# ethz-asl/multipoint

Measured on AMD Instinct MI355X. Metric: image-pairs/sec (detect+desc+match) @ 480x640, higher is better.
Workload: dtype f32

## Files before the change

multipoint_amd/csrc/api.hip:

```cpp
#include "host.h"

using namespace mp_host;

namespace {

bool debug_switch(const char* key, int* value = nullptr, int dflt = 1)
{
    const char* e = getenv("MP_DEBUG");
    if (!e) return false;
    const size_t kl = std::strlen(key);
    for (const char* q = e; *q;) {
        while (*q == ',' || *q == ' ') ++q;
        const char* end = q;
        while (*end && *end != ',') ++end;
        if ((size_t)(end - q) >= kl && std::strncmp(q, key, kl) == 0 && (q[kl] == '=' || q + kl == end || q[kl] == ' ')) {
            if (value) *value = q[kl] == '=' ? atoi(q + kl + 1) : dflt;
            return true;
        }
        q = end;
    }
    return false;
}

int kfd_num_xcc(const char* bus_id)
// ... 69 lines not shown
        char bus[64] = {0};
        if (hipDeviceGetPCIBusId(bus, sizeof bus, device) == hipSuccess) nxcd = kfd_num_xcc(bus);
        if (nxcd <= 0) nxcd = ncu >= 32 ? ncu / 32 : 1;
        int v = 0;
        if (debug_switch("ncu", &v) && v > 0 && v <= ncu) ncu = v;
        if (debug_switch("nxcd", &v) && v > 0) nxcd = v;
    }
    if (ncu < 1 || nxcd < 1 || (nxcd & (nxcd - 1)) != 0 || nxcd > ncu)
        return fail(h, MP_EINVAL, "mp_create: unsupported machine shape: " + std::to_string(ncu) + " compute units in " +
                                      std::to_string(nxcd) + " XCDs (the XCD count must be a power of two <= the CU count)");
    int xcd_shift = 0;
    while ((1 << xcd_shift) < nxcd) ++xcd_shift;
    DebugSwitches d;
    int v = 0;
    d.winograd = !debug_switch("no_winograd");
    if (debug_switch("wino43", &v) && v == 0) d.wino43 = false;
    if (debug_switch("wino43_gen", &v) && v >= 0 && v <= 2) d.wino43_gen = v;
    d.fuse_first = !debug_switch("no_fuse");
    d.fuse43 = !debug_switch("no_fuse43");
    d.head_fuse = !debug_switch("no_head_fuse");
    d.vin = !debug_switch("no_vin");
    d.planar = !debug_switch("no_planar");
    d.xplanar = d.planar && !debug_switch("no_xplanar");
    if (debug_switch("persist_min_items", &v) && v > 0) d.persist = v;
    if (debug_switch("no_persist")) d.persist = 0;
    if (debug_switch("splitk_max", &v) && v >= 1 && v <= 8) d.splitk_max = v;
    d.f16_res = !debug_switch("f16_no_res");
    d.f16_fuse1 = !debug_switch("f16_no_fuse1");
    if (debug_switch("f16_res_groups", &v) && v == 2) d.f16_res_groups = 2;
    mp_handle* hh = new mp_handle(device, ncu, xcd_shift, d);
    if (hipHostMalloc(reinterpret_cast<void**>(&hh->pinned), 4096) != hipSuccess) {
        delete hh;
        return fail(h, MP_ENOMEM, "mp_create: hipHostMalloc failed");
    }
    *out = hh;
    return MP_OK;
}

void mp_destroy(mp_handle* h)
{
    if (!h) return;
    (void)hipSetDevice(h->device);
    int* pinned = h->pinned;
    const std::vector<ProfEntry> events = std::move(h->prof_entries);
    delete h;
    if (pinned) (void)hipHostFree(pinned);
// ... 31 lines not shown
```

multipoint_amd/csrc/conv_wino43.hip:

```cpp
#include "mp_common.h"
#include "mp_device.h"
#include "mp_tile.h"

#include <algorithm>
#include <type_traits>

MP_TIMING_TABLE(g_timing_q, 256 * 8, mp_debug_read_timing_wino43)
MP_TIMING_HEIGHT(g_timing_q_sel, 480, mp_debug_select_height_wino43)

namespace {

constexpr int NPIX = 18 * 34;
constexpr int UC4 = 4;
constexpr int VB4 = UC4 * 32 * 36;
constexpr int UB4 = UC4 * 64 * 36;
constexpr int NRB = (NPIX + 63) / 64;
constexpr int RB4 = NRB * 64 * 4;
constexpr int SW4 = 8 * 36 * 2;


template <int LEAD = 0>
__device__ __forceinline__ void dma16(const float* sbase, unsigned voff_bytes, unsigned lds_byte)
{
    lds_dma<4, LEAD, 0>(sbase, voff_bytes, lds_byte);
}

template <bool POOL, bool BNF, int TC4, bool F1, bool SPLIT = false, bool VIN = false>
__global__ __launch_bounds__(512, 2) void conv_wino43_kernel(const ConvParams p)
{
    static_assert(!(F1 && SPLIT), "the fused first block is never split");
    static_assert(!(VIN && (F1 || SPLIT)), "pre-transformed input: plain launches only");
    constexpr int TR4 = 32 / TC4;
    constexpr int OY = 4 * TR4, OX = 4 * TC4;
    constexpr int PY = OY + 2, PX = OX + 2;
    static_assert(PY * PX == NPIX, "item shape");
    __shared__ __attribute__((aligned(16))) float Vs[(VIN ? 4 : 2) * VB4];
    __shared__ __attribute__((aligned(16))) float Us[2 * UB4];
    __shared__ __attribute__((aligned(16))) float raw[VIN ? 256 : 3 * RB4 + 256];
    __shared__ __attribute__((aligned(16))) float scr[VIN ? 4 : 8 * SW4];
    __shared__ __attribute__((aligned(16))) float prm[(POOL && !SPLIT ? 6 : 3) * 64];

    const int tid = threadIdx.x;
    const int lane = tid & 63;
    const int wave = __builtin_amdgcn_readfirstlane(tid >> 6);
    const int tb = wave & 1, cb = wave >> 1;
    const int NC = SPLIT ? (p.cin / UC4) >> p.ks_shift : p.cin / UC4;

    const XcdRange xr = xcd_range(p.nitems, p.xcd_shift);
    const int stride = xr.stride, item_end = xr.item_end;
    int item = xr.item;
    if (item >= item_end) return;

    struct Where { int slice, img, y0, x0, tile; const float* in_base; };
    auto decode = [&](int it) __attribute__((always_inline)) -> Where {
        Where w{};
        const int tile = (int)udiv((unsigned)it, p.magic_slices, (unsigned)p.nslices);
        w.slice = it - tile * p.nslices;
        w.tile = tile;
        const int trow = (int)udiv((unsigned)tile, p.magic_tx, (unsigned)p.tiles_x);
        const int tx = tile - trow * p.tiles_x;
        const int bi = (int)udiv((unsigned)trow, p.magic_ty, (unsigned)p.tiles_y);
        const int ty = trow - bi * p.tiles_y;
        w.img = p.img_list ? p.img_list[bi] : bi;
        w.y0 = ty * OY; w.x0 = tx * OX;
        w.in_base = p.in_planar ? p.in + (long long)w.img * (p.cin / 4) * p.H * p.W * 4
                                : p.in + (long long)w.img * p.H * p.W * p.in_cstride + p.in_coff;
        if constexpr (SPLIT)
            w.in_base += (long long)((w.slice & ((1 << p.ks_shift) - 1)) * NC) * (p.in_planar ? (long long)p.H * p.W * 4 : UC4);
        return w;
    };

    const int pix_stride = p.in_planar ? 4 : p.in_cstride;
    const long long unit_stride = p.in_planar ? (long long)p.H * p.W * 4 : UC4;
    const int x_shift = p.in_planar == MP_LAYOUT_XPLANAR ? 2 : 0, x_mask = p.in_planar == MP_LAYOUT_XPLANAR ? 3 : 0;
    const int row_stride = p.W * pix_stride;
    auto pixel_off = [&](int y, int x) __attribute__((always_inline)) -> int {
        return y * row_stride + (x >> x_shift) * pix_stride + (x & x_mask) * p.W;
    };
    unsigned rvoff[2];
    bool roff_rel = false;
    auto raw_offsets = [&](const Where& w) __attribute__((always_inline)) -> const float* {
// ... 447 lines not shown
                unit(c + 2, std::false_type{}, VB1{}, VS3{});
                unit(c + 3, std::false_type{}, VB0{}, VB0{});
            }
            unit(NC - 3, std::false_type{}, VB1{}, VB1{});
            unit(NC - 2, std::false_type{}, VB0{}, VS2{});
            unit(NC - 1, std::false_type{}, VB1{}, VS3{});
        } else {
        unit(0, std::true_type{}, VB0{}, VB0{});
        for (int c = 1; c + 1 < NC; c += 2) {
            unit(c, std::false_type{}, VB1{}, VB1{});
            unit(c + 1, std::false_type{}, VB0{}, VB0{});
        }
        unit(NC - 1, std::false_type{}, VB1{}, VB1{});
        }

        MP_CLOCK(t_e0);
        MP_CLOCK_ADD(3, t_item, t_e0);
        if constexpr (F1) { if (item_next + stride < item_end) patch_dma(decode(item_next + stride), cur_par); }
        const int tl = tb * 16 + (lane & 15);
        const int cl = cb * 16 + 4 * (lane >> 4);
        const f32x4 b4 = *reinterpret_cast<const f32x4*>(&prm[cl]);
        const f32x4 s4 = *reinterpret_cast<const f32x4*>(&prm[64 + cl]);
        const f32x4 t4 = *reinterpret_cast<const f32x4*>(&prm[128 + cl]);
        const int oy = cur.y0 + 4 * (tl / TC4), ox = cur.x0 + 4 * (tl % TC4);
        const int ch0 = (SPLIT ? cur.slice >> p.ks_shift : cur.slice) * 64 + cl;
        const int cs = p.out_cstride;
        constexpr int NO = POOL ? 2 : 4;
        f32x2 keep[NO][NO];
        if constexpr (SPLIT) {
            unsigned long long* const part = reinterpret_cast<unsigned long long*>(p.split_scratch) + (long long)item * (2 * 16 * 512) + tid;
#pragma unroll
            for (int h = 0; h < 2; ++h) {
                f32x2 tcol[4][6];
#pragma unroll
                for (int j = 0; j < 6; ++j) {
                    f32x2 m[6], y[4];
#pragma unroll
                    for (int i = 0; i < 6; ++i) m[i] = f32x2{acc[6 * i + j][2 * h], acc[6 * i + j][2 * h + 1]};
                    at6s(m, y);
#pragma unroll
                    for (int a = 0; a < 4; ++a) tcol[a][j] = y[a];
                }
#pragma unroll
                for (int a = 0; a < 4; ++a) {
                    f32x2 y[4];
                    at6s(tcol[a], y);
#pragma unroll
// ... 62 lines not shown
            for (int a = 0; a < 4; ++a) {
                f32x2 y[4];
                at6s(tcol[a], y);
#pragma unroll
                for (int b = 0; b < 4; ++b) {
                    f32x2 v = w43_add_bias(y[b], a, b, bb);
                    if (BNF) { v = v * ss + tt; v = f32x2{relu_bits(v[0]), relu_bits(v[1])}; }
                    else { v = f32x2{relu_bits(v[0]), relu_bits(v[1])}; v = v * ss + tt; }
                    yv[a][b] = v;
                }
            }
#pragma unroll
            for (int a = 0; a < NO; ++a)
#pragma unroll
                for (int b = 0; b < NO; ++b) res[a][b] = yv[a][b];
            }
            if (h == 0) {
#pragma unroll
                for (int a = 0; a < NO; ++a)
#pragma unroll
                    for (int b = 0; b < NO; ++b) keep[a][b] = res[a][b];
            } else {
                const int Ho = POOL ? p.H >> 1 : p.H, Wo = POOL ? p.W >> 1 : p.W;
                const int py0 = POOL ? oy >> 1 : oy, px0 = POOL ? ox >> 1 : ox;
                const bool xpl = !POOL && p.out_planar == MP_LAYOUT_XPLANAR;
                char* const img_base = reinterpret_cast<char*>(
                    p.out_planar ? p.out + (long long)cur.img * (p.cout / 4) * Ho * Wo * 4
                                 : p.out + (long long)cur.img * Ho * Wo * cs + p.out_coff);
                const unsigned ps = xpl ? (unsigned)Wo * 4u : p.out_planar ? 16u : (unsigned)cs * 4u;
                const unsigned rs = p.out_planar ? (unsigned)Wo * 16u : (unsigned)Wo * ps;
                const unsigned o0 = xpl ? (unsigned)(((ch0 >> 2) * Ho + py0) * Wo * 4 + px0) * 4u
                                  : p.out_planar ? (unsigned)(((ch0 >> 2) * Ho + py0) * Wo + px0) * 16u
                                                 : (unsigned)((py0 * Wo + px0) * cs + ch0) * 4u;
                if (oy < p.H && ox < p.W && ch0 < p.cout) {
#pragma unroll
                    for (int a = 0; a < NO; ++a)
#pragma unroll
                        for (int b = 0; b < NO; ++b) {
                            const f32x4 v = {keep[a][b][0], keep[a][b][1], res[a][b][0], res[a][b][1]};
                            *reinterpret_cast<f32x4*>(img_base + (o0 + (unsigned)a * rs + (unsigned)b * ps)) = v;
                        }
                }
            }
        }
        }
        MP_CLOCK(t_e1);
        MP_CLOCK_ADD(2, t_e0, t_e1);
#ifdef MP_TIMING
        tsum[7] += 1;
        if (!has_next && tid == 0 && t_on)
            for (int i = 0; i < 8; ++i) g_timing_q[blockIdx.x * 8 + i] = tsum[i];
#endif
        if (!has_next) { dma_wait(); return; }
        if (next_slice != cur.slice) {
            __syncthreads();
            load_prm(next_slice);
        }
        item = item_next;
        cur = decode(item);
        cur_par ^= 1;
        up = unext;
    }
}

template <int TC4>
__global__ __launch_bounds__(256) void wino43_vprod_kernel(const ConvParams p, long long ntb)
{
    constexpr int TR4 = 32 / TC4, OY = 4 * TR4, OX = 4 * TC4;
    __shared__ __attribute__((aligned(16))) float st[19456];
    const int ncp = p.cin >> 1, NC = p.cin / UC4;
    const int TL = 256 / ncp;
    const int RS = TL * 36 + 4;
    const int groups = 32 / TL;
    const int tid = threadIdx.x;
    const int cp = tid % ncp, tlc = tid / ncp;
    const long long tb = (long long)blockIdx.x / groups;
    const int t0 = ((int)((long long)blockIdx.x % groups)) * TL, t = t0 + tlc;
    (void)ntb;
    const int tx = (int)(tb % p.tiles_x);
    const long long trow = tb / p.tiles_x;
    const int ty = (int)(trow % p.tiles_y);
    const int bi = (int)(trow / p.tiles_y);
    const int img = p.img_list ? p.img_list[bi] : bi;
    const int wy = ty * OY + 4 * (t / TC4) - 1, wx = tx * OX + 4 * (t % TC4) - 1;
    const float* const base = p.in + (long long)img * p.H * p.W * p.in_cstride + p.in_coff + 2 * cp;
    int gx[6];
#pragma unroll
    for (int j = 0; j < 6; ++j) gx[j] = reflect_clamp(wx + j, p.W);
    f32x2 r[6][6];
#pragma unroll
    for (int j = 0; j < 6; ++j) {
        f32x2 d[6], o[6];
#pragma unroll
        for (int i = 0; i < 6; ++i)
            d[i] = *reinterpret_cast<const f32x2*>(base + ((long long)reflect_clamp(wy + i, p.H) * p.W + gx[j]) * p.in_cstride);
        bt6(d, o);
#pragma unroll
        for (int i = 0; i < 6; ++i) r[i][j] = o[i];
    }
    float* const dst0 = st + (2 * cp) * RS + tlc * 36;
    float* const dst1 = dst0 + RS;
#pragma unroll
    for (int i = 0; i < 6; i += 2) {
        f32x2 a[6], b[6];
        bt6(r[i], a);
        bt6(r[i + 1], b);
        *reinterpret_cast<f32x4*>(dst0 + 6 * i) = f32x4{a[0][0], a[1][0], a[2][0], a[3][0]};
// ... 9 lines not shown
    for (int i = tid; i < total4; i += 256) {
        const int row = i / q4, w = i - row * q4;
        *reinterpret_cast<f32x4*>(gbase + (long long)row * (32 * 36) + w * 4) = *reinterpret_cast<const f32x4*>(st + row * RS + w * 4);
    }
}

template <bool POOL, int TC4, bool F1 = false, bool SPLIT = false>
int launch_q(const ConvParams& p, hipStream_t s)
{
    constexpr int OY = 4 * (32 / TC4), OX = 4 * TC4;
    ConvParams q = p;
    if (SPLIT) q.nslices = p.nslices << p.ks_shift;
    q.tiles_x = (p.W + OX - 1) / OX; q.tiles_y = (p.H + OY - 1) / OY;
    const long long nitems = (long long)p.B * q.tiles_x * q.tiles_y * q.nslices;
    if (nitems <= 0) return 0;
    if (tile_items(q, nitems)) return 1;
    const unsigned grid = persistent_grid(nitems, p.ncu, p.xcd_shift);
    const ConvParams& pp = q;
    if (p.bn_first) hipLaunchKernelGGL((conv_wino43_kernel<POOL, true, TC4, F1, SPLIT>), dim3(grid), dim3(512), 0, s, pp);
    else hipLaunchKernelGGL((conv_wino43_kernel<POOL, false, TC4, F1, SPLIT>), dim3(grid), dim3(512), 0, s, pp);
    return 0;
}

template <int TC4>
int launch_vin(const ConvParams& p, hipStream_t s)
{
    constexpr int OY = 4 * (32 / TC4), OX = 4 * TC4;
    ConvParams q = p;
    q.tiles_x = (p.W + OX - 1) / OX; q.tiles_y = (p.H + OY - 1) / OY;
    const long long ntb = (long long)p.B * q.tiles_x * q.tiles_y, nitems = ntb * q.nslices;
    if (nitems <= 0) return 0;
    if (tile_items(q, nitems)) return 1;
    const ConvParams& pp = q;
    const int tl = 256 / (p.cin / 2);
    hipLaunchKernelGGL((wino43_vprod_kernel<TC4>), dim3((unsigned)(ntb * (32 / tl))), dim3(256), 0, s, pp, ntb);
    const unsigned grid = persistent_grid(nitems, p.ncu, p.xcd_shift);
    if (p.bn_first) hipLaunchKernelGGL((conv_wino43_kernel<false, true, TC4, false, false, true>), dim3(grid), dim3(512), 0, s, pp);
    else hipLaunchKernelGGL((conv_wino43_kernel<false, false, TC4, false, false, true>), dim3(grid), dim3(512), 0, s, pp);
    return 0;
}

template <bool POOL, bool SPLIT = false>
int launch_shape(const ConvParams& p, hipStream_t s)
{
    const long long wide = (long long)((p.W + 31) / 32) * ((p.H + 15) / 16), tall = (long long)((p.W + 15) / 16) * ((p.H + 31) / 32);
    return tall < wide ? launch_q<POOL, 4, false, SPLIT>(p, s) : launch_q<POOL, 8, false, SPLIT>(p, s);
}

}

bool conv_wino43_supports(const ConvParams& p)
{
    return !p.pad_zero && p.cin % 8 == 0 && p.cout % 4 == 0 && p.H % 4 == 0 && p.W % 4 == 0 && p.H >= 4 && p.W >= 4 &&
           p.in_cstride % 4 == 0 && p.in_coff % 4 == 0 && p.out_cstride % 4 == 0 && p.out_coff % 4 == 0;
}

long long conv_wino43_vglobal_floats(const ConvParams& p)
{
    const long long wide = (long long)((p.W + 31) / 32) * ((p.H + 15) / 16), tall = (long long)((p.W + 15) / 16) * ((p.H + 31) / 32);
    return (long long)p.B * std::min(wide, tall) * (p.cin / UC4) * VB4;
}

long long conv_wino43_items(const ConvParams& p)
{
    const long long wide = (long long)((p.W + 31) / 32) * ((p.H + 15) / 16), tall = (long long)((p.W + 15) / 16) * ((p.H + 31) / 32);
    return (long long)p.B * std::min(wide, tall) * p.nslices;
}

int launch_conv_wino43(const ConvParams& p, bool pool, hipStream_t s, bool fuse_first)
{
    if (p.out_planar == MP_LAYOUT_XPLANAR && pool) return 2;
    if ((p.in_planar == MP_LAYOUT_XPLANAR || p.out_planar == MP_LAYOUT_XPLANAR) && p.ks_shift > 0) return 2;
    if (fuse_first) return pool && p.cin == 64 ? launch_q<true, 8, true>(p, s) : 2;
    if (p.vglobal) {
        if (pool || p.ks_shift > 0 || p.cin % 16 != 0 || p.in_planar || p.cin > 256 || 256 % (p.cin / 2) != 0 || (p.cin / 2) < 8) return 2;
        const long long wide = (long long)((p.W + 31) / 32) * ((p.H + 15) / 16), tall = (long long)((p.W + 15) / 16) * ((p.H + 31) / 32);
        return tall < wide ? launch_vin<4>(p, s) : launch_vin<8>(p, s);
    }
    if (p.ks_shift > 0) {
        const int ncs = (p.cin / 4) >> p.ks_shift;
        if (ncs < 4 || (ncs & 1) || (ncs << p.ks_shift) * 4 != p.cin || !p.split_scratch) return 2;
        const int rc = pool ? launch_shape<true, true>(p, s) : launch_shape<false, true>(p, s);
        return rc ? rc : launch_split_reduce(p, 1, pool, s);
    }
    return pool ? launch_shape<true>(p, s) : launch_shape<false>(p, s);
}
```

multipoint_amd/csrc/forward.hip:

```cpp
#include "host.h"

using namespace mp_host;

namespace {

int pick_mbw(int H, int W)
{
    long long best = -1;
    int arg = 32;
    for (int mbw : {32, 16, 8}) {
        const int tw = mbw, th = 256 / mbw;
        const long long area = (long long)((H + th - 1) / th) * th * ((W + tw - 1) / tw) * tw;
        if (best < 0 || area < best) { best = area; arg = mbw; }
    }
    return arg;
}

void prof_begin(mp_handle* h, const char* name, double flop, hipStream_t s)
{
    if (!h->prof) return;
    if (h->prof_used == h->prof_entries.size()) {
        ProfEntry e{};
        (void)hipEventCreate(&e.a); (void)hipEventCreate(&e.b);
        h->prof_entries.push_back(e);
// ... 9 lines not shown
    (void)hipEventRecord(h->prof_entries[h->prof_used].b, s);
    ++h->prof_used;
}

int launch_failed(mp_handle* h, int code, const char* name, int B, int H, int W)
{
    const std::string layer = std::string("mp_forward: layer ") + name;
    if (code == 1)
        return fail(h, MP_EINVAL, layer + " has too many work items for one launch (B=" + std::to_string(B) + ", " +
                                      std::to_string(H) + "x" + std::to_string(W) + "): split the batch");
    return fail(h, MP_EINVAL, layer + ": the selected convolution kernel does not cover this layer shape (" + std::to_string(H) +
                                  "x" + std::to_string(W) + ")");
}


enum class Kernel { direct, wino43, wino43b, f16, f16_res, f16_res_slices };

struct ConvLaunch {
    Kernel kernel = Kernel::direct;
    bool fuse_first = false;
    int in_planar = MP_LAYOUT_NHWC, out_planar = MP_LAYOUT_NHWC;
    int ks_shift = 0;
    bool vin = false;
};

struct EncoderPlan { ConvLaunch conv[7]; };

Kernel wino43_kind(const mp_handle* h, const ConvLayer& L, int H, int W, int in_cstride, int in_coff, int out_cstride, int out_coff)
{
    if (!(L.taps == 9 && L.u43pack && h->policy.wino43)) return Kernel::direct;
    ConvParams q{};
    q.pad_zero = h->cfg.reflection_pad ? 0 : 1; q.cin = L.cin; q.cout = L.cout; q.H = H; q.W = W;
    q.in_cstride = in_cstride; q.in_coff = in_coff; q.out_cstride = out_cstride; q.out_coff = out_coff;
    if (h->policy.wino43_gen != 2 && conv_wino43_supports(q)) return Kernel::wino43;
    if (h->policy.wino43_gen != 1 && conv_wino43b_supports(q)) return Kernel::wino43b;
    return Kernel::direct;
}

void plan_split_vin(const mp_handle* h, const ConvLayer& L, int B, int H, int W, int fwd_batch, ConvLaunch& c)
{
    if ((c.kernel != Kernel::wino43 && c.kernel != Kernel::wino43b) || c.fuse_first) return;
    if (fwd_batch <= 2 && h->policy.splitk_max > 1) {
        ConvParams q{};
        q.B = B; q.H = H; q.W = W; q.nslices = L.nslices;
        const long long items = conv_wino43_items(q);
        const int units = L.cin / 4;
        int ks = 0;
        while ((items << (ks + 1)) <= h->ncu && (2 << ks) <= h->policy.splitk_max && (units >> (ks + 1)) >= 4 &&
               ((units >> (ks + 1)) & 1) == 0 && ((units >> (ks + 1)) << (ks + 1)) == units) ++ks;
        if (ks > 0 && items <= 1024) c.ks_shift = ks;
    }
    c.vin = c.kernel == Kernel::wino43 && !L.pool && c.ks_shift == 0 && !c.in_planar && L.cin % 16 == 0 && L.cin <= 256 &&
            256 % (L.cin / 2) == 0 && L.cin >= 16 && h->dbg.vin && L.nslices >= 4;
}

Kernel f16_kind(const mp_handle* h, const ConvLayer& L, int in_cstride, int in_coff, bool fuse_first)
{
    ConvParamsH q{};
    q.cin = L.cin; q.cout = L.cout; q.nslices = L.nslices; q.in_cstride = in_cstride; q.in_coff = in_coff;
    if (h->dbg.f16_res && conv_f16_res_supports(q, L.taps)) return Kernel::f16_res;
    if (h->dbg.f16_res && !fuse_first && L.taps == 9 && L.cin == 64 && L.nslices > 1 && L.cout == 64 * L.nslices)
        return Kernel::f16_res_slices;
    return Kernel::f16;
}

EncoderPlan plan_encoder(const mp_handle* h, const Encoder& E, int nb, int fwd_batch, int H, int W)
{
    EncoderPlan P;
    if (h->cfg.mixed_precision) {
        const ConvLayer& L0 = E.conv[0];
        P.conv[0].fuse_first = h->dbg.f16_res && h->dbg.f16_fuse1 && h->cfg.reflection_pad && !E.first_pool && L0.pool &&
                               L0.cin == 64 && L0.cout == 64 && L0.nslices == 1;
        for (int i = 0; i < E.nconv; ++i) P.conv[i].kernel = f16_kind(h, E.conv[i], E.conv[i].cin, 0, P.conv[i].fuse_first);
        return P;
    }
    for (int i = 0, hh = E.first_pool ? H / 2 : H, ww = E.first_pool ? W / 2 : W; i < E.nconv; ++i) {
// ... 51 lines not shown
    p.scale = L.scale; p.shift = L.shift; p.img_list = img_list;
    if (c.fuse_first) {
        p.img = images; p.w1 = f16 ? first->w_h : first->w; p.b1 = f16 ? first->bias_h : first->bias;
        p.s1 = first->scale; p.t1 = first->shift;
    }
    if constexpr (f16) {
        p.wpack = L.wpack_h; p.bias = L.bias_h;
        p.dummy = static_cast<_Float16*>(h->f16_dummy.p);
        p.res_groups = h->dbg.f16_res_groups;
    } else {
        p.wpack = c.kernel == Kernel::direct ? L.wpack : L.u43pack; p.bias = L.bias;
        p.relu = L.relu ? 1 : 0;
        p.persist = h->dbg.persist;
        p.in_planar = c.in_planar; p.out_planar = c.out_planar;
        if (c.fuse_first && c.kernel != Kernel::direct) {
            p.wpack = L.u43pack_f1; p.bias = L.bias_f1; p.w1 = first->w_f1; p.b1 = first->bias_f1; p.s1 = nullptr; p.t1 = nullptr;
        }
        if (c.ks_shift) {
            const int rc = ensure(h, h->split_ws, (size_t)(conv_wino43_items(p) << c.ks_shift) * (2 * 16 * 512 * 8));
            if (rc) return rc;
            p.ks_shift = c.ks_shift; p.split_scratch = static_cast<float*>(h->split_ws.p);
        }
        if (c.vin) {
            if (ensure(h, h->vin_ws, (size_t)conv_wino43_vglobal_floats(p) * 4) == MP_OK) p.vglobal = static_cast<float*>(h->vin_ws.p);
            else { (void)hipGetLastError(); h->err.clear(); }
        }
    }
    prof_begin(h, c.fuse_first ? "enc.conv1+2" : L.name,
               2.0 * L.taps * L.cin * L.cout * (double)B * H * W + (c.fuse_first ? 2.0 * 9 * 64 * (double)B * H * W : 0.0), s);
    int big = 0;
    if constexpr (f16) {
        if (c.kernel == Kernel::f16_res) {
            big = launch_conv_f16_res(p, mbw, L.pool, s);
        } else if (c.kernel == Kernel::f16_res_slices) {
            for (int sl = 0; sl < L.nslices && !big; ++sl) {
                ConvParamsH q = p;
                q.wpack = p.wpack + (size_t)sl * 36 * 2 * 64 * 8;
                q.bias = p.bias + 64 * sl; q.scale = p.scale + 64 * sl; q.shift = p.shift + 64 * sl;
                q.out_coff = out_coff + 64 * sl; q.cout = 64; q.nslices = 1;
                big = conv_f16_res_supports(q, L.taps) ? launch_conv_f16_res(q, mbw, L.pool, s) : 2;
            }
        } else {
            big = launch_conv_f16(p, L.taps, mbw, L.pool, s);
        }
    } else {
        big = c.kernel == Kernel::wino43b ? launch_conv_wino43b(p, L.pool, s)
// ... 85 lines not shown
        for (int i = 0; i < E.nconv; ++i) {
            const ConvLayer& L = E.conv[i];
            if ((rc = run_conv(h, L, plan.conv[i], src, L.cin, 0, i == E.nconv - 1 ? X : dst, L.cout, 0, nb, hh, ww, list, s,
                               &E.first, images))) return rc;
            if (L.pool) { hh /= 2; ww /= 2; }
            T* t = src; src = dst; dst = t;
        }
    }

    const int Hc = H / 8, Wc = W / 8, lstride = f16 ? 128 : 80;
    const long long npx = (long long)B * Hc * Wc;
    const int D = h->cfg.descriptor_size;
    const int hc = h->head_channels;
    const int headc = h->cfg.descriptor_head ? 2 * hc : hc;
    const int encc = h->heads3.cin;
    ConvLaunch c3, c1x1;
    if constexpr (f16) {
        c3.kernel = f16_kind(h, h->heads3, encc, 0, false);
        c1x1.kernel = Kernel::f16;
    } else {
        c3.kernel = wino43_kind(h, h->heads3, Hc, Wc, encc, 0, headc, 0);
        plan_split_vin(h, h->heads3, B, Hc, Wc, B, c3);
    }
    if ((rc = run_conv(h, h->heads3, c3, X, encc, 0, P, headc, 0, B, Hc, Wc, nullptr, s))) return rc;
    if (h->dbg.head_fuse && (!f16 || prob || logits || desc)) {
        typename std::conditional<f16, HeadTailParamsH, HeadTailParams>::type t{};
        t.x = P; t.xstride = headc; t.K = hc;
        if constexpr (f16) {
            t.wdet = h->det1.wpack_h; t.bdet = h->det1.bias_h; t.wdesc = h->desc1.wpack_h; t.bdesc = h->desc1.bias_h;
        } else {
            t.wdet = h->det1.wpack; t.bdet = h->det1.bias; t.wdesc = h->desc1.wpack; t.bdesc = h->desc1.bias;
        }
        t.sdet = h->det1.scale; t.tdet = h->det1.shift; t.sdesc = h->desc1.scale; t.tdesc = h->desc1.shift;
        t.D = D; t.npx = npx; t.B = B; t.Hc = Hc; t.Wc = Wc;
        t.prob = prob; t.logits_nchw = logits; t.desc = desc;
        t.softmax_mode = h->cfg.softmax_mode; t.normalize = h->cfg.normalize_descriptors ? 1 : 0; t.ncu = h->ncu;
        prof_begin(h, "heads.tail", 2.0 * hc * (65.0 + (desc ? D : 0)) * (double)npx, s);
        int miss;
        if constexpr (f16) miss = launch_head_tail_f16(t, s); else miss = launch_head_tail(t, s);
        prof_end(h, s);
        if (!miss) return launch_status(h);
        if (h->prof) --h->prof_used;
        if (!h->head_fallback_noted) {
            h->head_fallback_noted = true;
            fprintf(stderr, "[multipoint_hip] note: fused head tail not instantiated for %d head channels / descriptor size %d: "
                            "using the separate 1x1 convolution, softmax and normalisation launches\n", hc, D);
        }
    }
    if ((rc = run_conv(h, h->det1, c1x1, P, headc, 0, Lg, lstride, 0, B, Hc, Wc, nullptr, s))) return rc;
    if (prob || logits) {
        prof_begin(h, "det.softmax_shuffle", 0.0, s);
        if constexpr (f16) launch_det_post_f16(Lg, lstride, B, Hc, Wc, prob, logits, h->cfg.softmax_mode, s);
        else launch_det_post(Lg, lstride, B, Hc, Wc, prob, logits, h->cfg.softmax_mode, s);
        prof_end(h, s);
    }
    if (desc) {
        T* raw;
        if constexpr (f16) raw = R; else raw = desc;
// ... 246 lines not shown
```

multipoint_amd/csrc/head_tail.hip:

```cpp
#include "mp_common.h"
#include "mp_device.h"

#include <type_traits>

namespace {

__device__ __forceinline__ float acc_rd(float a)
{
    float x;
    asm volatile("v_accvgpr_read_b32 %0, %1" : "=v"(x) : "a"(a));
    return x;
}
template <int ND>
__global__ __launch_bounds__(256) void head_tail_kernel(const HeadTailParams p)
{
    constexpr int NT = 3 + ND;
    constexpr int NP = 96 + 32 * ND;
    constexpr int WCH = 4 * NT * 256;
    constexpr int XCH = 2 * 4 * 256;
    __shared__ __attribute__((aligned(16))) float wl[2 * WCH];
    __shared__ __attribute__((aligned(16))) float xl[2 * 4 * XCH];
    __shared__ __attribute__((aligned(16))) float prm[3 * NP];
    const int tid = threadIdx.x, lane = tid & 63;
    const int wave = __builtin_amdgcn_readfirstlane(tid >> 6);
    const int pl = lane & 31, hf = lane >> 5;
    for (int i = tid; i < NP; i += 256) {
        const bool det = i < 96;
        const int c = det ? i : i - 96;
        prm[i] = det ? p.bdet[c] : p.bdesc[c];
        prm[NP + i] = det ? p.sdet[c] : p.sdesc[c];
        prm[2 * NP + i] = det ? p.tdet[c] : p.tdesc[c];
    }

    const long long ntiles = (p.npx + 127) / 128;
    long long tile = blockIdx.x;
    long long px = 0;
    bool valid = false;
    unsigned xoff = 0, xoff_next = 0;
    const float *xbase = p.x, *xbase_next = p.x;
    auto place = [&](long long t, unsigned& off, const float*& base) __attribute__((always_inline)) {
        const long long q = (t * 4 + wave) * 32 + pl;
        off = (unsigned)(((q < p.npx ? q : p.npx - 1) - t * 128) * p.xstride + hf * 4) * 4u;
        base = p.x + t * 128 * p.xstride;
    };
    place(tile, xoff, xbase);
    const int nchunks = p.K >> 5;
    const unsigned wl_lds = (unsigned)(size_t)wl, xl_lds = (unsigned)(size_t)xl + (unsigned)wave * (XCH * 4u);

    auto chunk_dma = [&](int c, int buf, int j, bool next_tile) __attribute__((always_inline)) {
        if (j < NT) {
            const int nb = j < 3 ? j : j - 3;
            const float* w = j < 3 ? p.wdet : p.wdesc;
            const float* src = w + (((((long long)(nb >> 1) * nchunks + c) * 4 + wave) * 2 + (nb & 1)) * 64) * 4;
            lds_dma<4, 0, 0>(src, (unsigned)lane * 16u, wl_lds + (unsigned)(buf * WCH + (wave * NT + j) * 256) * 4u);
        } else {
            const int q = j - NT, part = q >> 2, g = q & 3;
            if (ND == 0 && part == 1) return;
            lds_dma<4, 0, 0>((next_tile ? xbase_next : xbase) + part * p.K + c * 32 + g * 8, next_tile ? xoff_next : xoff,
                             xl_lds + (unsigned)(buf * 4 * XCH + (part * 4 + g) * 256) * 4u);
        }
    };

#pragma unroll
    for (int j = 0; j < NT + 8; ++j) chunk_dma(0, 0, j, false);
    dma_wait();
    __syncthreads();

    for (;;) {
    const bool has_next = tile + gridDim.x < ntiles;
    if (has_next) place(tile + gridDim.x, xoff_next, xbase_next);
    px = (tile * 4 + wave) * 32 + pl;
    valid = px < p.npx;
    f32x16 acc[NT];
#pragma unroll
    for (int t = 0; t < NT; ++t)
#pragma unroll
        for (int r = 0; r < 16; ++r) acc[t][r] = 0.f;

    auto chunk = [&](int c, auto buf_tag, bool prefetch, bool next_tile) __attribute__((always_inline)) {
        constexpr int buf = decltype(buf_tag)::value;
        const float* const wb = wl + buf * WCH + lane * 4;
        const float* const xb = xl + wave * XCH + buf * 4 * XCH + lane * 4;
// ... 100 lines not shown
            if (p.normalize) {
                ss += __shfl_xor(ss, 32);
                const float rd = 1.0f / fmaxf(sqrtf(ss), 1e-12f);
#pragma unroll
                for (int i = 0; i < ND * 4; ++i) dv[i] = dv[i] * rd;
            }
            if (valid) {
                float* o = p.desc + px * (32 * ND) + 4 * hf;
#pragma unroll
                for (int t = 0; t < ND; ++t)
#pragma unroll
                    for (int q = 0; q < 4; ++q) *reinterpret_cast<f32x4*>(o + 32 * t + 8 * q) = dv[4 * t + q];
            }
        }
    }
    if (!has_next) return;
    tile += gridDim.x;
    xoff = xoff_next; xbase = xbase_next;
    }
}

}

int launch_head_tail(const HeadTailParams& p, hipStream_t s)
{
    if (p.K % 64 != 0 || p.npx <= 0) return 1;
    const int D = p.desc ? p.D : 0;
    const long long tiles = (p.npx + 127) / 128;
    const dim3 grid((unsigned)(tiles < p.ncu ? tiles : p.ncu)), block(256);
    switch (D) {
    case 0: hipLaunchKernelGGL(head_tail_kernel<0>, grid, block, 0, s, p); return 0;
    case 64: hipLaunchKernelGGL(head_tail_kernel<2>, grid, block, 0, s, p); return 0;
    case 128: hipLaunchKernelGGL(head_tail_kernel<4>, grid, block, 0, s, p); return 0;
    case 256: hipLaunchKernelGGL(head_tail_kernel<8>, grid, block, 0, s, p); return 0;
    default: return 1;
    }
}
```

multipoint_amd/csrc/host.h:

```cpp
#pragma once
#include "../../include/multipoint_hip.h"
#include "mp_common.h"

#include <cmath>
#include <cstdio>
#include <cstdlib>
#include <cstring>
#include <map>
#include <string>
#include <type_traits>
#include <vector>

namespace mp_host {

inline std::string g_create_error;

struct DevBuf {
    void* p = nullptr;
    size_t bytes = 0;
    DevBuf(void* p_ = nullptr, size_t bytes_ = 0) : p(p_), bytes(bytes_) {}
    DevBuf(DevBuf&& o) noexcept : p(o.p), bytes(o.bytes) { o.p = nullptr; o.bytes = 0; }
    ~DevBuf() { if (p) (void)hipFree(p); }
};

// ... 17 lines not shown

struct Encoder {
    FirstLayer first;
    ConvLayer conv[7];
    int nconv = 7;
    bool first_pool = false;
};

struct BnLayer {
    std::string name;
    int channels = 0;
    float *gamma = nullptr, *beta = nullptr;
    long long offset = 0;
};

struct ProfEntry {
    const char* name;
    hipEvent_t a, b;
    double flop;
};

struct DebugSwitches {
    bool winograd = true, wino43 = true, fuse_first = true, fuse43 = true, head_fuse = true, vin = true, planar = true;
    bool xplanar = true, f16_res = true, f16_fuse1 = true;
    int wino43_gen = 0, persist = 8, splitk_max = 8, f16_res_groups = 3;
};

struct ConvPolicy {
    bool direct = false;
    bool wino43 = true;
    int wino43_gen = 0;
    int splitk_max = 8;
};

struct MiRefine {
    void* workspace = nullptr;
    MiLaunch L{};
    int P = 0, normalized = 0;
    double sigma = 0.0;
    long long smooth_stride = 0;
    unsigned* counts = nullptr;
    float* warped = nullptr;
    double *smooth_a = nullptr, *smooth_b = nullptr, *cand = nullptr, *values = nullptr;
    const double* reg_init = nullptr;
    MiNmState* state = nullptr;
    int* nact = nullptr;
};
// ... 92 lines not shown
```

multipoint_amd/csrc/mp_common.h:

```cpp
#pragma once
#include <hip/hip_runtime.h>
#include <stdint.h>

typedef float f32x16 __attribute__((ext_vector_type(16)));
typedef float f32x4 __attribute__((ext_vector_type(4)));
typedef float f32x2 __attribute__((ext_vector_type(2)));

#define MP_WAVE 64

enum { MP_LAYOUT_NHWC = 0, MP_LAYOUT_PLANAR = 1, MP_LAYOUT_XPLANAR = 2 };

struct ConvParams {
    const float* in;
    float* out;
    const float* wpack;
    const float* bias;
    const float* scale;
    const float* shift;
    const int* img_list;
    const float* img;
    const float *w1, *b1, *s1, *t1;
    int B, H, W;
    int in_cstride, in_coff, cin;
    int out_cstride, out_coff, cout;
    int nslices;
    int tiles_x, tiles_y;
    int pad_zero;
    int bn_first;
    int relu;
    long long total_px;
    unsigned magic_slices, magic_tx, magic_ty;
    int nitems;
    int persist;
    int in_planar, out_planar;
    int ncu, xcd_shift;
    int ks_shift;
    float* split_scratch;
    float* vglobal;
};

struct XcdRange { int item, item_end, stride; };
__device__ __forceinline__ XcdRange xcd_range(int nitems, int xcd_shift)
{
    const int nxcd = 1 << xcd_shift;
    const int per_xcd = (nitems + nxcd - 1) >> xcd_shift;
    const int xcd = (int)blockIdx.x & (nxcd - 1);
    XcdRange r;
    r.stride = (int)gridDim.x >> xcd_shift;
    r.item_end = min((xcd + 1) * per_xcd, nitems);
    r.item = xcd * per_xcd + ((int)blockIdx.x >> xcd_shift);
    return r;
}
inline unsigned persistent_grid(long long nitems, int ncu, int xcd_shift, int per_cu = 1)
{
    const long long nxcd = 1ll << xcd_shift;
    const long long full = ((long long)ncu * per_cu) / nxcd * nxcd;
    const long long need = (nitems + nxcd - 1) / nxcd * nxcd;
    return (unsigned)(need < full ? need : full);
}

struct Conv1Params {
// ... 58 lines not shown
    r[4] = pk_fnma_k<1>(t3, K_AB, t2);
    r[5] = pk_fma_k<0>(d[1], K_PS, pk_fnma_k<1>(d[3], K_PS, d[5]));
}
static_assert(MP_W43_B == 2 * MP_W43_A, "at6s() needs b = 2a");
__device__ __forceinline__ void at6s(const f32x2 m[6], f32x2 z[4])
{
    constexpr float a3 = (float)(MP_W43_A * MP_W43_A * MP_W43_A);
    const f32x2 s1 = m[1] + m[2], d1 = m[1] - m[2], s2 = m[3] + m[4], d2 = m[3] - m[4];
    z[0] = (m[0] + s1) + s2;
    z[1] = __builtin_elementwise_fma(d2, f32x2{2.f, 2.f}, d1);
    z[2] = __builtin_elementwise_fma(s2, f32x2{4.f, 4.f}, s1);
    z[3] = __builtin_elementwise_fma(__builtin_elementwise_fma(d2, f32x2{8.f, 8.f}, d1), f32x2{a3, a3}, m[5]);
}
constexpr float w43_sigma(int r) { return r == 1 ? (float)MP_W43_A : r == 2 ? (float)(MP_W43_A * MP_W43_A) : 1.f; }
constexpr float w43_out_scale(int r, int c) { return w43_sigma(r) * w43_sigma(c); }
__device__ __forceinline__ f32x2 w43_add_bias(f32x2 z, int r, int c, f32x2 bias)
{
    const float k = w43_out_scale(r, c);
    return k == 1.f ? z + bias : __builtin_elementwise_fma(z, f32x2{k, k}, bias);
}
bool conv_wino43_supports(const ConvParams& p);
long long conv_wino43_items(const ConvParams& p);
long long conv_wino43_vglobal_floats(const ConvParams& p);
int launch_conv_wino43(const ConvParams& p, bool pool, hipStream_t s, bool fuse_first = false);
bool conv_wino43b_supports(const ConvParams& p);
int launch_conv_wino43b(const ConvParams& p, bool pool, hipStream_t s);
int launch_split_reduce(const ConvParams& p, int gen, bool pool, hipStream_t s);

struct ConvParamsH {
    const _Float16* in;
    _Float16* out;
    const _Float16* wpack;
    const float* bias;
    const float* scale;
    const float* shift;
    const int* img_list;
    int B, H, W;
    int in_cstride, in_coff, cin;
    int out_cstride, out_coff, cout;
    int nslices, tiles_x, tiles_y;
    int pad_zero, bn_first;
    long long total_px;
    unsigned magic_slices, magic_tx, magic_ty;
    int nitems;
    _Float16* dummy;
    int ncu, xcd_shift;
// ... 10 lines not shown
    int B, H, W;
    int pad_zero, bn_first;
    int pool;
};
int launch_conv_f16(const ConvParamsH& p, int taps, int mbw, bool pool, hipStream_t s);
bool conv_f16_res_supports(const ConvParamsH& p, int taps);
int launch_conv_f16_res(const ConvParamsH& p, int mbw, bool pool, hipStream_t s);
void launch_conv_first_f16(const Conv1ParamsH& p, hipStream_t s);

struct HeadTailParams {
    const float* x;
    int xstride, K;
    const float *wdet, *bdet, *sdet, *tdet;
    const float *wdesc, *bdesc, *sdesc, *tdesc;
    int D;
    long long npx;
    int B, Hc, Wc;
    float* prob;
    float* logits_nchw;
    float* desc;
    int softmax_mode;
    int normalize;
    int ncu;
};
int launch_head_tail(const HeadTailParams& p, hipStream_t s);
struct HeadTailParamsH {
    const _Float16* x;
    int xstride, K;
    const _Float16 *wdet, *wdesc;
    const float *bdet, *sdet, *tdet, *bdesc, *sdesc, *tdesc;
    int D;
    long long npx;
    int B, Hc, Wc;
    float* prob; float* logits_nchw; float* desc;
    int softmax_mode, normalize, ncu;
};
int launch_head_tail_f16(const HeadTailParamsH& p, hipStream_t s);
void launch_det_post(const float* logits, int lstride, int B, int Hc, int Wc, float* prob,
                     float* logits_nchw, int mode, hipStream_t s);
void launch_det_post_f16(const _Float16* logits, int lstride, int B, int Hc, int Wc, float* prob,
                         float* logits_nchw, int mode, hipStream_t s);
void launch_desc_l2norm(const float* raw, float* out, long long npx, int D, int normalize,
                        hipStream_t s);
void launch_desc_l2norm_f16(const _Float16* raw, float* out, long long npx, int D, int normalize,
                            hipStream_t s);

#define MP_NMS_MAX_R 15
struct NmsFootprint {
// ... 183 lines not shown
```

Measured before the change: 3528.

## Pack Winograd 4x4 tiles densely for head conv and emit xplanar output to tail

```diff
diff --git a/multipoint_amd/csrc/api.hip b/multipoint_amd/csrc/api.hip
--- a/multipoint_amd/csrc/api.hip
+++ b/multipoint_amd/csrc/api.hip
@@ -115,6 +115,7 @@
     d.vin = !debug_switch("no_vin");
     d.planar = !debug_switch("no_planar");
     d.xplanar = d.planar && !debug_switch("no_xplanar");
+    d.head_dense = !debug_switch("no_head_dense");
     if (debug_switch("persist_min_items", &v) && v > 0) d.persist = v;
     if (debug_switch("no_persist")) d.persist = 0;
     if (debug_switch("splitk_max", &v) && v >= 1 && v <= 8) d.splitk_max = v;
diff --git a/multipoint_amd/csrc/conv_wino43.hip b/multipoint_amd/csrc/conv_wino43.hip
--- a/multipoint_amd/csrc/conv_wino43.hip
+++ b/multipoint_amd/csrc/conv_wino43.hip
@@ -25,11 +25,12 @@
     lds_dma<4, LEAD, 0>(sbase, voff_bytes, lds_byte);
 }
 
-template <bool POOL, bool BNF, int TC4, bool F1, bool SPLIT = false, bool VIN = false>
+template <bool POOL, bool BNF, int TC4, bool F1, bool SPLIT = false, bool VIN = false, bool DENSE = false>
 __global__ __launch_bounds__(512, 2) void conv_wino43_kernel(const ConvParams p)
 {
     static_assert(!(F1 && SPLIT), "the fused first block is never split");
     static_assert(!(VIN && (F1 || SPLIT)), "pre-transformed input: plain launches only");
+    static_assert(!DENSE || (VIN && !POOL), "dense tile blocks: un-pooled pre-transformed launches only");
     constexpr int TR4 = 32 / TC4;
     constexpr int OY = 4 * TR4, OX = 4 * TC4;
     constexpr int PY = OY + 2, PX = OX + 2;
@@ -57,6 +58,7 @@
         const int tile = (int)udiv((unsigned)it, p.magic_slices, (unsigned)p.nslices);
         w.slice = it - tile * p.nslices;
         w.tile = tile;
+        if constexpr (DENSE) return w;
         const int trow = (int)udiv((unsigned)tile, p.magic_tx, (unsigned)p.tiles_x);
         const int tx = tile - trow * p.tiles_x;
         const int bi = (int)udiv((unsigned)trow, p.magic_ty, (unsigned)p.tiles_y);
@@ -550,7 +552,7 @@
         const f32x4 b4 = *reinterpret_cast<const f32x4*>(&prm[cl]);
         const f32x4 s4 = *reinterpret_cast<const f32x4*>(&prm[64 + cl]);
         const f32x4 t4 = *reinterpret_cast<const f32x4*>(&prm[128 + cl]);
-        const int oy = cur.y0 + 4 * (tl / TC4), ox = cur.x0 + 4 * (tl % TC4);
+        const int oy = DENSE ? 0 : cur.y0 + 4 * (tl / TC4), ox = DENSE ? 0 : cur.x0 + 4 * (tl % TC4);
         const int ch0 = (SPLIT ? cur.slice >> p.ks_shift : cur.slice) * 64 + cl;
         const int cs = p.out_cstride;
         constexpr int NO = POOL ? 2 : 4;
@@ -659,17 +661,30 @@
                     for (int b = 0; b < NO; ++b) keep[a][b] = res[a][b];
             } else {
                 const int Ho = POOL ? p.H >> 1 : p.H, Wo = POOL ? p.W >> 1 : p.W;
-                const int py0 = POOL ? oy >> 1 : oy, px0 = POOL ? ox >> 1 : ox;
+                int oy_l = oy, ox_l = ox;
+                unsigned img_off = 0u;
+                if constexpr (DENSE) {
+                    const unsigned T = (unsigned)cur.tile * 32u + (unsigned)tl;
+                    const bool live = T < (unsigned)(p.B * p.tiles_y * p.tiles_x);
+                    const unsigned Tc = live ? T : 0u;
+                    const unsigned trow = udiv(Tc, p.magic_tx, (unsigned)p.tiles_x);
+                    const unsigned bi = udiv(trow, p.magic_ty, (unsigned)p.tiles_y);
+                    ox_l = 4 * (int)(Tc - trow * (unsigned)p.tiles_x);
+                    oy_l = live ? 4 * (int)(trow - bi * (unsigned)p.tiles_y) : p.H;
+                    img_off = bi * ((unsigned)(Ho * Wo) * (p.out_planar ? (unsigned)p.cout : (unsigned)cs) * 4u);
+                }
+                const int py0 = POOL ? oy_l >> 1 : oy_l, px0 = POOL ? ox_l >> 1 : ox_l;
                 const bool xpl = !POOL && p.out_planar == MP_LAYOUT_XPLANAR;
                 char* const img_base = reinterpret_cast<char*>(
-                    p.out_planar ? p.out + (long long)cur.img * (p.cout / 4) * Ho * Wo * 4
-                                 : p.out + (long long)cur.img * Ho * Wo * cs + p.out_coff);
+                    DENSE ? p.out + (p.out_planar ? 0 : p.out_coff)
+                    : p.out_planar ? p.out + (long long)cur.img * (p.cout / 4) * Ho * Wo * 4
+                                   : p.out + (long long)cur.img * Ho * Wo * cs + p.out_coff);
                 const unsigned ps = xpl ? (unsigned)Wo * 4u : p.out_planar ? 16u : (unsigned)cs * 4u;
                 const unsigned rs = p.out_planar ? (unsigned)Wo * 16u : (unsigned)Wo * ps;
-                const unsigned o0 = xpl ? (unsigned)(((ch0 >> 2) * Ho + py0) * Wo * 4 + px0) * 4u
-                                  : p.out_planar ? (unsigned)(((ch0 >> 2) * Ho + py0) * Wo + px0) * 16u
-                                                 : (unsigned)((py0 * Wo + px0) * cs + ch0) * 4u;
-                if (oy < p.H && ox < p.W && ch0 < p.cout) {
+                const unsigned o0 = img_off + (xpl ? (unsigned)(((ch0 >> 2) * Ho + py0) * Wo * 4 + px0) * 4u
+                                               : p.out_planar ? (unsigned)(((ch0 >> 2) * Ho + py0) * Wo + px0) * 16u
+                                                              : (unsigned)((py0 * Wo + px0) * cs + ch0) * 4u);
+                if (oy_l < p.H && ox_l < p.W && ch0 < p.cout) {
 #pragma unroll
                     for (int a = 0; a < NO; ++a)
 #pragma unroll
@@ -700,8 +715,8 @@
     }
 }
 
-template <int TC4>
-__global__ __launch_bounds__(256) void wino43_vprod_kernel(const ConvParams p, long long ntb)
+template <int TC4, bool DENSE = false>
+__global__ __launch_bounds__(256) void wino43_vprod_kernel(const ConvParams p, long long ntiles)
 {
     constexpr int TR4 = 32 / TC4, OY = 4 * TR4, OX = 4 * TC4;
     __shared__ __attribute__((aligned(16))) float st[19456];
@@ -713,13 +728,21 @@
     const int cp = tid % ncp, tlc = tid / ncp;
     const long long tb = (long long)blockIdx.x / groups;
     const int t0 = ((int)((long long)blockIdx.x % groups)) * TL, t = t0 + tlc;
-    (void)ntb;
-    const int tx = (int)(tb % p.tiles_x);
-    const long long trow = tb / p.tiles_x;
-    const int ty = (int)(trow % p.tiles_y);
-    const int bi = (int)(trow / p.tiles_y);
+    int tx, ty, bi;
+    if constexpr (DENSE) {
+        const long long T64 = tb * 32 + t;
+        const unsigned T = (unsigned)(T64 < ntiles ? T64 : ntiles - 1);
+        const unsigned trow = udiv(T, p.magic_tx, (unsigned)p.tiles_x);
+        bi = (int)udiv(trow, p.magic_ty, (unsigned)p.tiles_y);
+        tx = (int)(T - trow * (unsigned)p.tiles_x); ty = (int)(trow - (unsigned)bi * (unsigned)p.tiles_y);
+    } else {
+        tx = (int)(tb % p.tiles_x);
+        const long long trow = tb / p.tiles_x;
+        ty = (int)(trow % p.tiles_y);
+        bi = (int)(trow / p.tiles_y);
+    }
     const int img = p.img_list ? p.img_list[bi] : bi;
-    const int wy = ty * OY + 4 * (t / TC4) - 1, wx = tx * OX + 4 * (t % TC4) - 1;
+    const int wy = DENSE ? 4 * ty - 1 : ty * OY + 4 * (t / TC4) - 1, wx = DENSE ? 4 * tx - 1 : tx * OX + 4 * (t % TC4) - 1;
     const float* const base = p.in + (long long)img * p.H * p.W * p.in_cstride + p.in_coff + 2 * cp;
     int gx[6];
 #pragma unroll
@@ -775,21 +798,22 @@
     return 0;
 }
 
-template <int TC4>
+template <int TC4, bool DENSE = false>
 int launch_vin(const ConvParams& p, hipStream_t s)
 {
-    constexpr int OY = 4 * (32 / TC4), OX = 4 * TC4;
+    constexpr int OY = DENSE ? 4 : 4 * (32 / TC4), OX = DENSE ? 4 : 4 * TC4;
     ConvParams q = p;
     q.tiles_x = (p.W + OX - 1) / OX; q.tiles_y = (p.H + OY - 1) / OY;
-    const long long ntb = (long long)p.B * q.tiles_x * q.tiles_y, nitems = ntb * q.nslices;
+    const long long ntiles = (long long)p.B * q.tiles_x * q.tiles_y;
+    const long long ntb = DENSE ? (ntiles + 31) / 32 : ntiles, nitems = ntb * q.nslices;
     if (nitems <= 0) return 0;
     if (tile_items(q, nitems)) return 1;
     const ConvParams& pp = q;
     const int tl = 256 / (p.cin / 2);
-    hipLaunchKernelGGL((wino43_vprod_kernel<TC4>), dim3((unsigned)(ntb * (32 / tl))), dim3(256), 0, s, pp, ntb);
+    hipLaunchKernelGGL((wino43_vprod_kernel<TC4, DENSE>), dim3((unsigned)(ntb * (32 / tl))), dim3(256), 0, s, pp, ntiles);
     const unsigned grid = persistent_grid(nitems, p.ncu, p.xcd_shift);
-    if (p.bn_first) hipLaunchKernelGGL((conv_wino43_kernel<false, true, TC4, false, false, true>), dim3(grid), dim3(512), 0, s, pp);
-    else hipLaunchKernelGGL((conv_wino43_kernel<false, false, TC4, false, false, true>), dim3(grid), dim3(512), 0, s, pp);
+    if (p.bn_first) hipLaunchKernelGGL((conv_wino43_kernel<false, true, TC4, false, false, true, DENSE>), dim3(grid), dim3(512), 0, s, pp);
+    else hipLaunchKernelGGL((conv_wino43_kernel<false, false, TC4, false, false, true, DENSE>), dim3(grid), dim3(512), 0, s, pp);
     return 0;
 }
 
@@ -808,16 +832,34 @@
            p.in_cstride % 4 == 0 && p.in_coff % 4 == 0 && p.out_cstride % 4 == 0 && p.out_coff % 4 == 0;
 }
 
-long long conv_wino43_vglobal_floats(const ConvParams& p)
-{
+bool conv_wino43_vin_dense(const ConvParams& p)
+{
+    if (!p.vin_dense || p.img_list || p.B <= 0 || p.H < 4 || p.W < 4 || p.H % 4 || p.W % 4) return false;
+    const long long px = (long long)p.B * p.H * p.W, ntb = (px / 16 + 31) / 32;
+    const long long dmax = std::max(std::max(p.W / 4, p.H / 4), p.nslices);
+    return px * std::max(p.out_cstride, p.cout) * 4 < 0x100000000ll && ntb * 32 * dmax < 0x100000000ll;
+}
+
+namespace {
+long long tile_blocks(const ConvParams& p)
+{
+    if (conv_wino43_vin_dense(p)) return ((long long)p.B * (p.H / 4) * (p.W / 4) + 31) / 32;
     const long long wide = (long long)((p.W + 31) / 32) * ((p.H + 15) / 16), tall = (long long)((p.W + 15) / 16) * ((p.H + 31) / 32);
-    return (long long)p.B * std::min(wide, tall) * (p.cin / UC4) * VB4;
-}
-
-long long conv_wino43_items(const ConvParams& p)
-{
-    const long long wide = (long long)((p.W + 31) / 32) * ((p.H + 15) / 16), tall = (long long)((p.W + 15) / 16) * ((p.H + 31) / 32);
-    return (long long)p.B * std::min(wide, tall) * p.nslices;
+    return (long long)p.B * std::min(wide, tall);
+}
+}
+
+long long conv_wino43_vglobal_floats(const ConvParams& p) { return tile_blocks(p) * (p.cin / UC4) * VB4; }
+
+long long conv_wino43_items(const ConvParams& p) { return tile_blocks(p) * p.nslices; }
+
+extern "C" int mp_debug_wino43_counts(int B, int H, int W, int cin, int cout, int dense, long long* items, long long* vglobal_floats)
+{
+    ConvParams q{};
+    q.B = B; q.H = H; q.W = W; q.cin = cin; q.cout = cout; q.out_cstride = cout; q.nslices = (cout + 63) / 64; q.vin_dense = dense;
+    if (items) *items = conv_wino43_items(q);
+    if (vglobal_floats) *vglobal_floats = conv_wino43_vglobal_floats(q);
+    return conv_wino43_vin_dense(q) ? 1 : 0;
 }
 
 int launch_conv_wino43(const ConvParams& p, bool pool, hipStream_t s, bool fuse_first)
@@ -827,6 +869,7 @@
     if (fuse_first) return pool && p.cin == 64 ? launch_q<true, 8, true>(p, s) : 2;
     if (p.vglobal) {
         if (pool || p.ks_shift > 0 || p.cin % 16 != 0 || p.in_planar || p.cin > 256 || 256 % (p.cin / 2) != 0 || (p.cin / 2) < 8) return 2;
+        if (conv_wino43_vin_dense(p)) return launch_vin<8, true>(p, s);
         const long long wide = (long long)((p.W + 31) / 32) * ((p.H + 15) / 16), tall = (long long)((p.W + 15) / 16) * ((p.H + 31) / 32);
         return tall < wide ? launch_vin<4>(p, s) : launch_vin<8>(p, s);
     }
diff --git a/multipoint_amd/csrc/forward.hip b/multipoint_amd/csrc/forward.hip
--- a/multipoint_amd/csrc/forward.hip
+++ b/multipoint_amd/csrc/forward.hip
@@ -55,6 +55,7 @@
     int in_planar = MP_LAYOUT_NHWC, out_planar = MP_LAYOUT_NHWC;
     int ks_shift = 0;
     bool vin = false;
+    bool dense = false;
 };
 
 struct EncoderPlan { ConvLaunch conv[7]; };
@@ -85,6 +86,7 @@
     }
     c.vin = c.kernel == Kernel::wino43 && !L.pool && c.ks_shift == 0 && !c.in_planar && L.cin % 16 == 0 && L.cin <= 256 &&
             256 % (L.cin / 2) == 0 && L.cin >= 16 && h->dbg.vin && L.nslices >= 4;
+    c.dense = c.vin && h->dbg.head_dense;
 }
 
 Kernel f16_kind(const mp_handle* h, const ConvLayer& L, int in_cstride, int in_coff, bool fuse_first)
@@ -182,6 +184,7 @@
             p.ks_shift = c.ks_shift; p.split_scratch = static_cast<float*>(h->split_ws.p);
         }
         if (c.vin) {
+            p.vin_dense = c.dense ? 1 : 0;
             if (ensure(h, h->vin_ws, (size_t)conv_wino43_vglobal_floats(p) * 4) == MP_OK) p.vglobal = static_cast<float*>(h->vin_ws.p);
             else { (void)hipGetLastError(); h->err.clear(); }
         }
@@ -313,18 +316,26 @@
         c3.kernel = wino43_kind(h, h->heads3, Hc, Wc, encc, 0, headc, 0);
         plan_split_vin(h, h->heads3, B, Hc, Wc, B, c3);
     }
+    typename std::conditional<f16, HeadTailParamsH, HeadTailParams>::type t{};
+    t.D = D; t.npx = npx; t.K = hc; t.desc = desc;
+    const bool fused_tail = h->dbg.head_fuse && (!f16 || prob || logits || desc);
+    if constexpr (!f16) {
+        ConvParams q{};
+        q.B = B; q.H = Hc; q.W = Wc; q.cout = headc; q.out_cstride = headc; q.nslices = h->heads3.nslices; q.vin_dense = c3.dense ? 1 : 0;
+        if (c3.dense && fused_tail && conv_wino43_vin_dense(q) && head_tail_supports(t)) c3.out_planar = MP_LAYOUT_XPLANAR;
+        t.x_layout = c3.out_planar;
+    }
     if ((rc = run_conv(h, h->heads3, c3, X, encc, 0, P, headc, 0, B, Hc, Wc, nullptr, s))) return rc;
-    if (h->dbg.head_fuse && (!f16 || prob || logits || desc)) {
-        typename std::conditional<f16, HeadTailParamsH, HeadTailParams>::type t{};
-        t.x = P; t.xstride = headc; t.K = hc;
+    if (fused_tail) {
+        t.x = P; t.xstride = headc;
         if constexpr (f16) {
             t.wdet = h->det1.wpack_h; t.bdet = h->det1.bias_h; t.wdesc = h->desc1.wpack_h; t.bdesc = h->desc1.bias_h;
         } else {
             t.wdet = h->det1.wpack; t.bdet = h->det1.bias; t.wdesc = h->desc1.wpack; t.bdesc = h->desc1.bias;
         }
         t.sdet = h->det1.scale; t.tdet = h->det1.shift; t.sdesc = h->desc1.scale; t.tdesc = h->desc1.shift;
-        t.D = D; t.npx = npx; t.B = B; t.Hc = Hc; t.Wc = Wc;
-        t.prob = prob; t.logits_nchw = logits; t.desc = desc;
+        t.B = B; t.Hc = Hc; t.Wc = Wc;
+        t.prob = prob; t.logits_nchw = logits;
         t.softmax_mode = h->cfg.softmax_mode; t.normalize = h->cfg.normalize_descriptors ? 1 : 0; t.ncu = h->ncu;
         prof_begin(h, "heads.tail", 2.0 * hc * (65.0 + (desc ? D : 0)) * (double)npx, s);
         int miss;
diff --git a/multipoint_amd/csrc/head_tail.hip b/multipoint_amd/csrc/head_tail.hip
--- a/multipoint_amd/csrc/head_tail.hip
+++ b/multipoint_amd/csrc/head_tail.hip
@@ -11,7 +11,7 @@
     asm volatile("v_accvgpr_read_b32 %0, %1" : "=v"(x) : "a"(a));
     return x;
 }
-template <int ND>
+template <int ND, bool XPL = false>
 __global__ __launch_bounds__(256) void head_tail_kernel(const HeadTailParams p)
 {
     constexpr int NT = 3 + ND;
@@ -38,8 +38,16 @@
     bool valid = false;
     unsigned xoff = 0, xoff_next = 0;
     const float *xbase = p.x, *xbase_next = p.x;
+    const long long cstep = XPL ? (long long)p.Hc * p.Wc : 1;
     auto place = [&](long long t, unsigned& off, const float*& base) __attribute__((always_inline)) {
         const long long q = (t * 4 + wave) * 32 + pl;
+        if constexpr (XPL) {
+            const unsigned plane = (unsigned)(p.Hc * p.Wc), qc = (unsigned)(q < p.npx ? q : p.npx - 1);
+            const unsigned img = qc / plane, cell = qc - img * plane, y = cell / (unsigned)p.Wc, x = cell - y * (unsigned)p.Wc;
+            off = (img * (unsigned)p.xstride * plane + (unsigned)hf * 4u * plane + y * (unsigned)p.Wc * 4u + (x & 3u) * (unsigned)p.Wc + (x >> 2) * 4u) * 4u;
+            base = p.x;
+            return;
+        }
         off = (unsigned)(((q < p.npx ? q : p.npx - 1) - t * 128) * p.xstride + hf * 4) * 4u;
         base = p.x + t * 128 * p.xstride;
     };
@@ -56,8 +64,12 @@
         } else {
             const int q = j - NT, part = q >> 2, g = q & 3;
             if (ND == 0 && part == 1) return;
-            lds_dma<4, 0, 0>((next_tile ? xbase_next : xbase) + part * p.K + c * 32 + g * 8, next_tile ? xoff_next : xoff,
-                             xl_lds + (unsigned)(buf * 4 * XCH + (part * 4 + g) * 256) * 4u);
+            if constexpr (XPL)
+                lds_dma<4, 0, 0>(p.x + (part * p.K + c * 32 + g * 8) * cstep, next_tile ? xoff_next : xoff,
+                                 xl_lds + (unsigned)(buf * 4 * XCH + (part * 4 + g) * 256) * 4u);
+            else
+                lds_dma<4, 0, 0>((next_tile ? xbase_next : xbase) + part * p.K + c * 32 + g * 8, next_tile ? xoff_next : xoff,
+                                 xl_lds + (unsigned)(buf * 4 * XCH + (part * 4 + g) * 256) * 4u);
         }
     };
 
@@ -204,17 +216,29 @@
 
 }
 
+bool head_tail_supports(const HeadTailParams& p)
+{
+    const int D = p.desc ? p.D : 0;
+    return p.K % 64 == 0 && p.npx > 0 && (D == 0 || D == 64 || D == 128 || D == 256);
+}
+
 int launch_head_tail(const HeadTailParams& p, hipStream_t s)
 {
-    if (p.K % 64 != 0 || p.npx <= 0) return 1;
+    if (!head_tail_supports(p)) return 1;
     const int D = p.desc ? p.D : 0;
     const long long tiles = (p.npx + 127) / 128;
     const dim3 grid((unsigned)(tiles < p.ncu ? tiles : p.ncu)), block(256);
+    const bool xpl = p.x_layout == MP_LAYOUT_XPLANAR;
+#define MP_TAIL(ND)                                                                         \
+    if (xpl) hipLaunchKernelGGL((head_tail_kernel<ND, true>), grid, block, 0, s, p);        \
+    else hipLaunchKernelGGL((head_tail_kernel<ND, false>), grid, block, 0, s, p);           \
+    return 0
     switch (D) {
-    case 0: hipLaunchKernelGGL(head_tail_kernel<0>, grid, block, 0, s, p); return 0;
-    case 64: hipLaunchKernelGGL(head_tail_kernel<2>, grid, block, 0, s, p); return 0;
-    case 128: hipLaunchKernelGGL(head_tail_kernel<4>, grid, block, 0, s, p); return 0;
-    case 256: hipLaunchKernelGGL(head_tail_kernel<8>, grid, block, 0, s, p); return 0;
+    case 0: MP_TAIL(0);
+    case 64: MP_TAIL(2);
+    case 128: MP_TAIL(4);
+    case 256: MP_TAIL(8);
     default: return 1;
     }
-}
+#undef MP_TAIL
+}
diff --git a/multipoint_amd/csrc/host.h b/multipoint_amd/csrc/host.h
--- a/multipoint_amd/csrc/host.h
+++ b/multipoint_amd/csrc/host.h
@@ -63,7 +63,7 @@
 
 struct DebugSwitches {
     bool winograd = true, wino43 = true, fuse_first = true, fuse43 = true, head_fuse = true, vin = true, planar = true;
-    bool xplanar = true, f16_res = true, f16_fuse1 = true;
+    bool xplanar = true, head_dense = true, f16_res = true, f16_fuse1 = true;
     int wino43_gen = 0, persist = 8, splitk_max = 8, f16_res_groups = 3;
 };
 
diff --git a/multipoint_amd/csrc/mp_common.h b/multipoint_amd/csrc/mp_common.h
--- a/multipoint_amd/csrc/mp_common.h
+++ b/multipoint_amd/csrc/mp_common.h
@@ -37,6 +37,7 @@
     int ks_shift;
     float* split_scratch;
     float* vglobal;
+    int vin_dense;
 };
 
 struct XcdRange { int item, item_end, stride; };
@@ -141,6 +142,7 @@
 bool conv_wino43_supports(const ConvParams& p);
 long long conv_wino43_items(const ConvParams& p);
 long long conv_wino43_vglobal_floats(const ConvParams& p);
+bool conv_wino43_vin_dense(const ConvParams& p);
 int launch_conv_wino43(const ConvParams& p, bool pool, hipStream_t s, bool fuse_first = false);
 bool conv_wino43b_supports(const ConvParams& p);
 int launch_conv_wino43b(const ConvParams& p, bool pool, hipStream_t s);
@@ -197,8 +199,10 @@
     int softmax_mode;
     int normalize;
     int ncu;
+    int x_layout;
 };
 int launch_head_tail(const HeadTailParams& p, hipStream_t s);
+bool head_tail_supports(const HeadTailParams& p);
 struct HeadTailParamsH {
     const _Float16* x;
     int xstride, K;
```

New measurement: 3552, median of 6. About the same (+0.7%).
